# danisotelo/qm_door

Measured on AMD Instinct MI355X. Metric: MPC+WBC cycles/sec (AlienGo+Z1, N=100), higher is better.
Workload: dtype f64

## Files before the change

### qm_door_amd/csrc/kernels/aux_kernels.h

```cpp
#pragma once
#include "layout.h"
#include "lq_kernel.h"

namespace qmk {

__global__ void __launch_bounds__(64) input_weight_kernel(const ProblemR* P, const real* zeros, real* Rw) {
  __shared__ real J[12 * 12];
  __shared__ real RJ[12 * 12];
  const int lane = threadIdx.x;
  const ModelR& md = P->model;
  const int dd = lane < AD_DIRS ? lane : AD_DIRS - 1;
  const AdIn in{P->settings.initial_state, zeros, P->settings.initial_state, dd, 0.0_r};
  FlowOut<Du, Du3, Du3> f;
  BaseMotion2<Du, Du3> bm;
  centroidalSweep2<Du, Du3, Du3>(
      md, P->settings.gravity, in,
      [&](int c, Vec3<Du>, Vec3<Du3> v) {
        if (lane >= 3 && lane < 15) { const int j = lane - 3; J[(3 * c + 0) * 12 + j] = v.x.e; J[(3 * c + 1) * 12 + j] = v.y.e; J[(3 * c + 2) * 12 + j] = v.z.e; }
      },
      [&](Vec3<Du>, const Mat3<Du>&) { return Vec3<Du3>(); }, f, bm);
  __syncthreads();
  const real* Rt = P->settings.R_task;
  for (int e = lane; e < 144; e += 64) {
    const int i = e / 12, j = e % 12;
// ... 124 lines not shown
    for (int q = 0; q < NB; ++q) {
      const int iu0 = min(idx[q], Np - 1), iu1 = min(idx[q] + 1, Np - 1);
      const real* pl = isU ? Up + (size_t(inst) * Np + iu0) * 30 : Xp + (size_t(inst) * (Np + 1) + idx[q]) * 30;
      const real* pr = isU ? Up + (size_t(inst) * Np + iu1) * 30 : Xp + (size_t(inst) * (Np + 1) + min(idx[q] + 1, last)) * 30;
      l[q] = pl[c]; r[q] = pr[c];
    }
    const real x0v = (x0 && isX) ? x0[size_t(inst) * 30 + c] : 0.0_r;
#pragma unroll
    for (int q = 0; q < NB; ++q) { QM_KEEP(l[q]); QM_KEEP(r[q]); }
#pragma unroll
    for (int q = 0; q < NB; ++q) {
      const int k = k0 + q;
      const real v = alpha[q] * l[q] + (1.0_r - alpha[q]) * r[q];
      if (k <= Nn && isX) warmX[(size_t(inst) * (Nn + 1) + k) * 30 + c] = (k == 0 && x0) ? x0v : v;
      else if (k < Nn && isU) warmU[(size_t(inst) * Nn + k) * 30 + c] = v;
    }
  }
}

__global__ void __launch_bounds__(64) policy_eval_kernel(int batch, int N, const real* tgrid, const real* X, const real* U, const int* modes, const real* tEval,
                                                         real* xOut, real* uOut, int* modeOut) {
  const int inst = blockIdx.x, lane = threadIdx.x;
  if (inst >= batch) return;
  const real* tg = tgrid + size_t(inst) * (N + 1);
  const real t = tEval[inst];
  int idx; real alpha;
  timeSegmentWave(tg, N + 1, t, lane, idx, alpha);
  const int kMode = gridCountBelow(tg + 1, N, t, lane);
  if (lane < 30) {
    const real* xl = X + (size_t(inst) * (N + 1) + idx) * 30;
    xOut[size_t(inst) * 30 + lane] = alpha * xl[lane] + (1.0_r - alpha) * xl[30 + lane];
  } else if (lane >= 32 && lane < 62) {
    const int i = lane - 32, iu0 = min(idx, N - 1), iu1 = min(idx + 1, N - 1);
    const real* ul = U + (size_t(inst) * N + iu0) * 30; const real* ur = U + (size_t(inst) * N + iu1) * 30;
    uOut[size_t(inst) * 30 + i] = alpha * ul[i] + (1.0_r - alpha) * ur[i];
  } else if (lane == 63) {
    modeOut[inst] = modes[size_t(inst) * (N + 1) + kMode];
  }
}

}
```

### qm_door_amd/csrc/kernels/linesearch_kernel.h

```cpp
#pragma once
#include "layout.h"
#include "schedule_dev.h"
#include "sweep_dev.h"

namespace qmk {

struct LsArgs {
  const ProblemR* P;
  const real* Rw;
  int batch, N, K, lineSearch;
  const real* eeContact;
  const real* tgrid; const real* dtgrid; const int* nodePhase;
  const real* X; const real* U; const real* dX; const real* dU;
  const real* targetTimes; const real* targetStates;
  const int* schedNum; const real* schedTimes; const int* schedModes;
  const real* metrics;
  const real* instStats;
  const int* nodeMode;
  real* Xt; real* Ut;
  real* outT; real* outX; real* outU; int* outMode; real* outStats;
  int iteration;
  int trialInLds;
  int* done;
};

constexpr int LS_STATIC_LDS_BYTES = (3 * 256 + 8 + 1800) * int(sizeof(real)) + int(sizeof(ModelR)) + 256 * 4 + 256;
inline int lsTrialLdsBytes(int N, int threads = 256) {
  const int trials = (N + 1 <= threads / 2) ? 2 : 1;
  const long long need = (long long)trials * (2 * N + 1) * 30 * (long long)sizeof(real);
  return need + LS_STATIC_LDS_BYTES <= 160 * 1024 ? int(need) : 0;
}
inline int lsThreads(int B, int N, int cus) { return (B > cus && N + 1 <= 128) ? 128 : 256; }

struct DblIn {
  const real* x; const real* u; real dtS; const real* k1;
  __device__ __forceinline__ real hn(int i) const { return x[i] + dtS * k1[i]; }
  __device__ __forceinline__ real euler(int i) const { return x[9 + i] + dtS * k1[9 + i]; }
  __device__ __forceinline__ real q(int j) const { return x[12 + j] + dtS * u[12 + j]; }
  __device__ __forceinline__ real qd(int j) const { return u[12 + j]; }
  __device__ __forceinline__ Vec3<real> force(int c) const { return Vec3<real>(u[3 * c], u[3 * c + 1], u[3 * c + 2]); }
};

template <class WP> __device__ __attribute__((noinline)) void nodePerformance(const ModelR& md, const SettingsR& st, WP Qw, WP Rw, int weightStructure, const real* bc, const Schedule& sched, const real* tTimes, const real* tStates, const real* contact, int K, real t, real dt, int phase,
                                       bool terminal, const real* x, const real* u, const real* xnext, real& cost, real& dyn, real& eq, real* xnOut = nullptr) {
  QM_TICK_DECL;
  const int mode = sched.modes[phase];
  real eePosRef[3], eeQuatRef[4];
  eeReference(tTimes, tStates, K, t, eePosRef, eeQuatRef);
  real Ke = 0.0_r, fRef[3] = {0.0_r, 0.0_r, 0.0_r}, pEnv[3] = {0.0_r, 0.0_r, 0.0_r};
  if (contact && !terminal) { Ke = st.ee_contact_stiffness; eeContactReference(tTimes, contact, K, t, fRef, pEnv); }
// ... 112 lines not shown
#pragma unroll
    for (int q = 0; q < UN; ++q) { const int e = base + q * stride, ec = e < n ? e : first; xv[q] = x[ec]; dv[q] = dx[ec]; }
#pragma unroll
    for (int q = 0; q < UN; ++q) { QM_KEEP(xv[q]); QM_KEEP(dv[q]); }
#pragma unroll
    for (int q = 0; q < UN; ++q) { const int e = base + q * stride; if (e < n) out[e] = alpha == 0.0_r ? xv[q] : xv[q] + alpha * dv[q]; }
  }
}
__device__ __forceinline__ real sumSquaresStrided(const real* v, int n, int first, int stride) {
  constexpr int UN = 8;
  real s = 0.0_r;
  for (int base = first; base < n; base += UN * stride) {
    real t[UN];
#pragma unroll
    for (int q = 0; q < UN; ++q) { const int e = base + q * stride; t[q] = v[e < n ? e : first]; }
#pragma unroll
    for (int q = 0; q < UN; ++q) QM_KEEP(t[q]);
#pragma unroll
    for (int q = 0; q < UN; ++q) { const int e = base + q * stride; if (e < n) s += t[q] * t[q]; }
  }
  return s;
}

#ifdef QM_RICCATI_TIMING
#define QM_LS_CLOCK(slot) do { const unsigned long long n_ = clock64(); if (blockIdx.x == 0 && threadIdx.x == 0) qmk::qmRiccatiTicks[240 + (slot)] += n_ - lsClk; lsClk = n_; } while (0)
#else
#define QM_LS_CLOCK(slot)
#endif
#if defined(QM_LS_EXTERN) && !defined(QM_RICCATI_TIMING)
__global__ void __launch_bounds__(256) linesearch_kernel(LsArgs a);
#else
__global__ void __launch_bounds__(256) linesearch_kernel(LsArgs a) {
#ifdef QM_RICCATI_TIMING
  unsigned long long lsClk = clock64();
#endif
  __shared__ real red[3 * 256];
  __shared__ real ctl[8];
  __shared__ int structVotes[256];
  __shared__ ModelR mdS;
  __shared__ __attribute__((aligned(16))) real wQ[900], wR[900];
  const int inst = blockIdx.x, tid = threadIdx.x, nthr = blockDim.x;
  if (a.done[inst]) return;
  const int N = a.N;
  const SettingsR& st = a.P->settings;
  const real* tg = a.tgrid + size_t(inst) * (N + 1);
  const Schedule sched{a.schedNum[inst], a.schedTimes + size_t(inst) * QMGPU_MAX_EVENTS, a.schedModes + size_t(inst) * (QMGPU_MAX_EVENTS + 1)};
  const real* tTimes = a.targetTimes + size_t(inst) * a.K;
  const real* tStates = a.targetStates + size_t(inst) * a.K * QMGPU_NTARGET;
  const real* X = a.X + size_t(inst) * (N + 1) * 30; const real* U = a.U + size_t(inst) * N * 30;
  const real* dX = a.dX + size_t(inst) * (N + 1) * 30; const real* dU = a.dU + size_t(inst) * N * 30;
  const int half = (N + 1 <= nthr / 2) ? nthr / 2 : nthr;
  const int nTr = nthr / half, myTr = tid / half, ltid = tid - myTr * half;
  QM_DYNAMIC_LDS(trialLds);
  real* Xt = a.trialInLds ? trialLds + size_t(myTr) * (2 * N + 1) * 30 : a.Xt + (size_t(inst) * 2 + myTr) * (N + 1) * 30;
  real* Ut = a.trialInLds ? Xt + (N + 1) * 30 : a.Ut + (size_t(inst) * 2 + myTr) * N * 30;

  constexpr int MDW = (int(sizeof(ModelR) / 4) + 255) / 256;
  int mdw[2 * MDW];
  const int mdPer = nthr >= 256 ? MDW : 2 * MDW;
  real m0 = 0.0_r, d0 = 0.0_r, e0 = 0.0_r;
  {
    bool outside = false;
    real qv[4], rv4[4];
#pragma unroll
    for (int q4 = 0; q4 < 4; ++q4) { const int e = tid + q4 * nthr, ec = e < 900 ? e : tid; qv[q4] = st.Q[ec]; rv4[q4] = a.Rw[ec]; }
    {
      const int* src = reinterpret_cast<const int*>(&a.P->model);
#pragma unroll
      for (int w = 0; w < 2 * MDW; ++w) { const int e = tid + w * nthr; mdw[w] = (w < mdPer && e < int(sizeof(ModelR) / 4)) ? src[e] : 0; }
    }
    real mk[3] = {0.0_r, 0.0_r, 0.0_r};
    if (tid <= N) { const real* m = a.metrics + (size_t(inst) * (N + 1) + tid) * NODE_METRICS; mk[0] = m[0]; mk[1] = m[1]; mk[2] = m[2]; }
#pragma unroll
    for (int q4 = 0; q4 < 4; ++q4) { QM_KEEP(qv[q4]); QM_KEEP(rv4[q4]); }
#pragma unroll
    for (int w = 0; w < 2 * MDW; ++w) QM_KEEP(mdw[w]);
    QM_KEEP(mk[0]); QM_KEEP(mk[1]); QM_KEEP(mk[2]);
    if (tid <= N) { m0 = mk[0]; d0 = mk[1]; e0 = mk[2]; }
#pragma unroll
    for (int q4 = 0; q4 < 4; ++q4) {
      const int e = tid + q4 * nthr;
      if (e < 900) {
        const real q = qv[q4], r = rv4[q4];
        wQ[e] = q; wR[e] = r;
        const int i = e / 30, j = e - 30 * i;
        const bool legBlock = i >= 12 && i < 24 && j >= 12 && j < 24;
        outside = outside || (i != j && q != 0.0_r) || (i != j && !legBlock && r != 0.0_r);
      }
    }
    for (int e = tid + 4 * nthr; e < 900; e += nthr) {
      const real q = st.Q[e], r = a.Rw[e];
      wQ[e] = q; wR[e] = r;
      const int i = e / 30, j = e - 30 * i;
      const bool legBlock = i >= 12 && i < 24 && j >= 12 && j < 24;
      outside = outside || (i != j && q != 0.0_r) || (i != j && !legBlock && r != 0.0_r);
    }
    structVotes[tid] = outside ? 1 : 0;
  }
  {
    int* dst = reinterpret_cast<int*>(&mdS);
#pragma unroll
    for (int w = 0; w < 2 * MDW; ++w) { const int e = tid + w * nthr; if (w < mdPer && e < int(sizeof(ModelR) / 4)) dst[e] = mdw[w]; }
  }
  for (int k = tid + nthr; k <= N; k += nthr) { const real* m = a.metrics + (size_t(inst) * (N + 1) + k) * NODE_METRICS; m0 += m[0]; d0 += m[1]; e0 += m[2]; }
  red[tid] = m0; red[256 + tid] = d0; red[512 + tid] = e0;
  __syncthreads();
  if (tid == 0) {
    real s0 = 0, s1 = 0, s2 = 0;
    int dense = 0;
    const int nSum = N + 1 < nthr ? N + 1 : nthr;
    for (int i = 0; i < nSum; ++i) { s0 += red[i]; s1 += red[256 + i]; s2 += red[512 + i]; }
    for (int i = 0; i < nthr; ++i) dense |= structVotes[i];
    ctl[0] = s0; ctl[1] = sqrt(s1 + s2); ctl[7] = dense ? 0.0_r : 1.0_r;
  }
  __syncthreads();
  QM_LS_CLOCK(0);
  const real merit0 = ctl[0], viol0 = ctl[1];
  const int weightStructure = int(ctl[7]);
  const real armijo = a.instStats[size_t(inst) * 4 + 0];
  const real ricStatus = a.instStats[size_t(inst) * 4 + 1];

  real alpha = 1.0_r, merit1 = merit0, viol1 = viol0;
  int stepType = 0;
  bool accepted = false;
#pragma unroll 1
  for (int trial = 0; trial < (ricStatus == 0.0_r ? 64 : 0); ++trial) {
    const real alphaMine = myTr ? alpha * st.alpha_decay : alpha;
    axpyStrided(Xt, X, dX, alphaMine, (N + 1) * 30, ltid, half);
    axpyStrided(Ut, U, dU, alphaMine, N * 30, ltid, half);
    __syncthreads();
    QM_LS_CLOCK(1);
    real cs = 0.0_r, ds = 0.0_r, es = 0.0_r;
    for (int k = ltid; k <= N; k += half) {
      real c, d, e;
      const bool term = k == N;
      nodePerformance(mdS, st, QM_TO_LDS_PTR(real, wQ), QM_TO_LDS_PTR(real, wR), weightStructure, a.Rw + QM_RW_DERIVED, sched, tTimes, tStates, a.eeContact ? a.eeContact + size_t(inst) * a.K * 6 : nullptr, a.K, tg[k], a.dtgrid[size_t(inst) * (N + 1) + k], a.nodePhase[size_t(inst) * (N + 1) + k], term, Xt + k * 30, term ? Ut : Ut + k * 30, term ? Xt + k * 30 : Xt + (k + 1) * 30, c, d, e);
      cs += c; ds += d; es += e;
    }
    QM_LS_CLOCK(2);
    red[tid] = cs; red[256 + tid] = ds; red[512 + tid] = es;
    __syncthreads();
    QM_LS_CLOCK(3);
    if (tid == 0) {
      real acc = 0.0_r, accAlpha = alpha, m1 = merit0, v1 = viol0; int type = 0;
      for (int tr = 0; tr < nTr && acc == 0.0_r; ++tr) {
        const real al = tr ? alpha * st.alpha_decay : alpha;
        if (tr && al < st.alpha_min) break;
        real s0 = 0, s1 = 0, s2 = 0;
        const int nTrial = N + 1 < half ? N + 1 : half;
        for (int i = tr * half; i < tr * half + nTrial; ++i) { s0 += red[i]; s1 += red[256 + i]; s2 += red[512 + i]; }
        m1 = s0; v1 = sqrt(s1 + s2);
        bool ok;
        if (!a.lineSearch) { ok = true; type = 0; }
        else if (v1 > st.g_max) { ok = v1 < (1.0_r - st.gamma_c) * viol0; type = 1; }
        else if (v1 < st.g_min && viol0 < st.g_min && al * armijo < 0.0_r) { ok = m1 < merit0 + st.armijo_factor * al * armijo; type = 3; }
        else { ok = m1 < merit0 - st.gamma_c * viol0 || v1 < (1.0_r - st.gamma_c) * viol0; type = 2; }
        accAlpha = al;
        if (ok) acc = 1.0_r;
      }
      ctl[2] = m1; ctl[3] = v1; ctl[4] = acc; ctl[5] = real(type); ctl[6] = accAlpha;
    }
    __syncthreads();
    QM_LS_CLOCK(4);
    merit1 = ctl[2]; viol1 = ctl[3]; stepType = int(ctl[5]);
    accepted = ctl[4] != 0.0_r;
    const real lastAlpha = ctl[6];
    __syncthreads();
    if (accepted) { alpha = lastAlpha; break; }
    alpha = lastAlpha * st.alpha_decay;
    if (alpha < st.alpha_min) break;
  }
  if (!accepted) { alpha = 0.0_r; stepType = 4; merit1 = merit0; viol1 = viol0; }
  real* oX = a.outX + size_t(inst) * (N + 1) * 30; real* oU = a.outU + size_t(inst) * N * 30;
  axpyStrided(oX, X, dX, alpha, (N + 1) * 30, tid, nthr);
  axpyStrided(oU, U, dU, alpha, N * 30, tid, nthr);
  for (int k = tid; k <= N; k += nthr) { a.outT[size_t(inst) * (N + 1) + k] = tg[k]; a.outMode[size_t(inst) * (N + 1) + k] = a.nodeMode[size_t(inst) * (N + 1) + k]; }
  QM_LS_CLOCK(5);
  const real sx = sumSquaresStrided(dX, (N + 1) * 30, tid, nthr), su = sumSquaresStrided(dU, N * 30, tid, nthr);
  __syncthreads();
  red[tid] = sx; red[256 + tid] = su;
  __syncthreads();
  if (tid == 0) {
    real s0 = 0, s1 = 0;
    for (int i = 0; i < nthr; ++i) { s0 += red[i]; s1 += red[256 + i]; }
    int conv = 0;
    if (a.iteration + 1 >= st.sqp_iterations) conv = 1;
    else if (alpha < st.alpha_min) conv = 2;
    else if (fabs(merit1 - merit0) < st.cost_tol && viol1 < st.g_min) conv = 3;
    else if (alpha * sqrt(s0) < st.delta_tol && alpha * sqrt(s1) < st.delta_tol) conv = 4;
    if (ricStatus != 0.0_r && conv == 0) conv = 2;
    a.done[inst] = conv;
    if (a.outStats) {
      real* s = a.outStats + size_t(inst) * QMGPU_NSTATS;
      s[0] = merit0; s[1] = viol0; s[2] = merit1; s[3] = viol1; s[4] = alpha; s[5] = real(stepType); s[6] = armijo; s[7] = ricStatus;
      s[8] = real(a.iteration + 1); s[9] = real(conv);
    }
  }
  QM_LS_CLOCK(6);
}
#endif

}
```

### qm_door_amd/csrc/kernels/mpc_pipeline.h

```cpp
#pragma once
#include <vector>

#include "aux_kernels.h"
#include "ddp_kernel.h"
#include "gpu_rt.h"
#include "layout.h"
#include "linesearch_kernel.h"
#include "lq_kernel.h"
#include "riccati_kernel.h"

namespace qmk {

struct MpcBuffers {
  ProblemR* dP = nullptr;
  real *dRw = nullptr, *dZeros = nullptr;
  real *dTgrid = nullptr, *dDtgrid = nullptr, *dX = nullptr, *dU = nullptr, *dStages = nullptr, *dAdRows = nullptr, *dMetrics = nullptr, *dGains = nullptr, *ddX = nullptr, *ddU = nullptr;
  real *dXt = nullptr, *dUt = nullptr, *dInstStats = nullptr, *dDebug = nullptr;
  int *dStageNc = nullptr, *dNodeMode = nullptr, *dNodePhase = nullptr, *dDone = nullptr;
  real *dDdpX = nullptr, *dDdpU = nullptr, *dDdpMerit = nullptr;
  int cus = 256;
};

struct MpcIo {
  int batch, N, K, lineSearch;
  double dtD;
  const double *t0D, *timeGridD, *schedTimesD;
  const real *x0, *targetTimes, *targetStates;
  const int* schedNum; const real* schedTimes; const int* schedModes;
  const real *warmX, *warmU;
  real *outT, *outX, *outU; int* outMode; real* outStats;
  const real* eeContact;
  int algorithm;
};

template <class Alloc> inline void allocateMpcBuffers(MpcBuffers& m, size_t B, size_t N, Alloc&& alloc) {
  const size_t N1 = N + 1;
  auto R = [&](size_t n, bool scratch = true) { return static_cast<real*>(alloc(n, sizeof(real), scratch)); };
  auto I = [&](size_t n) { return static_cast<int*>(alloc(n, sizeof(int), true)); };
  m.dP = static_cast<ProblemR*>(alloc(1, sizeof(ProblemR), false));
  m.dRw = R(QM_RW_DOUBLES, false);
  m.dZeros = R(64, false);
  m.dTgrid = R(B * N1);
  m.dDtgrid = R(B * N1);
  m.dNodePhase = I(B * N1);
  m.dX = R(B * N1 * 30);
  m.dU = R(B * N * 30);
  m.dStages = R(B * N1 * STAGE_DOUBLES);
  m.dAdRows = R(B * N1 * AD_DOUBLES);
  m.dMetrics = R(B * N1 * NODE_METRICS);
  m.dGains = R(B * N * GAIN_DOUBLES);
  m.ddX = R(B * N1 * 30);
  m.ddU = R(B * N * 30);
  m.dXt = R(2 * B * N1 * 30);
  m.dUt = R(2 * B * N * 30);
  m.dInstStats = R(B * 4);
  m.dStageNc = I(B * N1);
  m.dNodeMode = I(B * N1);
  m.dDone = I(B);
  int dev = 0, cus = 0;
  if (hipGetDevice(&dev) == hipSuccess && hipDeviceGetAttribute(&cus, hipDeviceAttributeMultiprocessorCount, dev) == hipSuccess && cus > 0) m.cus = cus;
}

template <class Alloc> inline void ensureDdpBuffers(MpcBuffers& m, size_t B, size_t N, Alloc&& alloc) {
  if (m.dDdpX) return;
  m.dDdpX = static_cast<real*>(alloc(size_t(DDP_MAX_TRIALS) * B * (N + 1) * 30, sizeof(real), true));
  m.dDdpU = static_cast<real*>(alloc(size_t(DDP_MAX_TRIALS) * B * N * 30, sizeof(real), true));
  m.dDdpMerit = static_cast<real*>(alloc(size_t(DDP_MAX_TRIALS) * B * 2, sizeof(real), true));
}

inline hipError_t prepareMpcKernels() {
  const hipError_t e = QM_ALLOW_DYNAMIC_LDS(riccati_kernel<RICCATI_WAVES>, RICCATI_LDS_BYTES);
  return e != hipSuccess ? e : QM_ALLOW_DYNAMIC_LDS(linesearch_kernel, 160 * 1024 - LS_STATIC_LDS_BYTES);
}

inline void enqueueMpcKernels(hipStream_t s, const MpcBuffers& m, const MpcIo& io, int iterations, bool debugLq, hipEvent_t* ev) {
  const int B = io.batch, N = io.N;
  if (ev) (void)hipEventRecord(ev[0], s);
  for (int it = 0; it < iterations; ++it) {
    InitArgs ia{m.dP, B, N, io.dtD, io.t0D, io.timeGridD, io.schedTimesD, io.x0, it == 0 ? io.warmX : io.outX, it == 0 ? io.warmU : io.outU, io.schedNum, io.schedModes,
                m.dTgrid, m.dDtgrid, m.dNodePhase, m.dX, m.dU, it, m.dDone};
    QM_LAUNCH(mpc_init_kernel, B, 128, s, ia);
    LqArgs la{m.dP, m.dRw, B, N, io.K, m.dTgrid, m.dDtgrid, m.dNodePhase, m.dX, m.dU, io.targetTimes, io.targetStates, io.schedNum, io.schedTimes,
              io.schedModes, m.dZeros, m.dStages, m.dStageNc, m.dNodeMode, m.dMetrics, debugLq ? m.dDebug : nullptr, m.dAdRows, m.dDone, io.eeContact};
    QM_LAUNCH(ad_node_kernel, adGridFor(B * (N + 1)), 64, s, la);
    if (ev) (void)hipEventRecord(ev[6], s);
    QM_LAUNCH(lq_node_kernel, B * (N + 1), 64, s, la);
    if (ev) (void)hipEventRecord(ev[1], s);
    RiccatiArgs ra{B, N, m.dStages, m.dStageNc, m.dDtgrid, io.x0, m.dX, m.dGains, m.ddX, m.ddU, m.dInstStats, m.dDone};
    QM_LAUNCH_DYN(riccati_kernel<RICCATI_WAVES>, B, RICCATI_WAVES * 64, RICCATI_LDS_BYTES, s, ra);
    if (ev) (void)hipEventRecord(ev[2], s);
    LsArgs ls{m.dP, m.dRw, B, N, io.K, io.lineSearch, io.eeContact, m.dTgrid, m.dDtgrid, m.dNodePhase, m.dX, m.dU, m.ddX, m.ddU, io.targetTimes, io.targetStates, io.schedNum,
              io.schedTimes, io.schedModes, m.dMetrics, m.dInstStats, m.dNodeMode, m.dXt, m.dUt, io.outT, io.outX, io.outU, io.outMode, io.outStats, it, lsTrialLdsBytes(N, lsThreads(B, N, m.cus)) > 0, m.dDone};
    QM_LAUNCH_DYN(linesearch_kernel, B, lsThreads(B, N, m.cus), lsTrialLdsBytes(N, lsThreads(B, N, m.cus)), s, ls);
    if (ev) (void)hipEventRecord(ev[3], s);
  }
}

inline void enqueueDdpKernels(hipStream_t s, const MpcBuffers& m, const MpcIo& io, int trials, hipEvent_t* ev) {
  const int B = io.batch, N = io.N;
  if (ev) (void)hipEventRecord(ev[0], s);
  InitArgs ia{m.dP, B, N, io.dtD, io.t0D, io.timeGridD, io.schedTimesD, io.x0, io.warmX, io.warmU, io.schedNum, io.schedModes, m.dTgrid, m.dDtgrid, m.dNodePhase, m.dX, m.dU, 0, m.dDone};
  QM_LAUNCH(mpc_init_kernel, B, 128, s, ia);
  DdpArgs ra{m.dP, m.dRw, B, N, io.K, 0, io.eeContact, m.dTgrid, m.dDtgrid, m.dNodePhase, io.x0, m.dX, m.dU, io.targetTimes, io.targetStates, io.schedNum, io.schedTimes, io.schedModes,
             m.dStages, m.dStageNc, m.dGains, m.dX, m.dU, m.dDdpMerit};
  if (!io.warmX) QM_LAUNCH(ddp_rollout_kernel, (B + 63) / 64, 64, s, ra);
  LqArgs la{m.dP, m.dRw, B, N, io.K, m.dTgrid, m.dDtgrid, m.dNodePhase, m.dX, m.dU, io.targetTimes, io.targetStates, io.schedNum, io.schedTimes,
            io.schedModes, m.dZeros, m.dStages, m.dStageNc, m.dNodeMode, m.dMetrics, nullptr, m.dAdRows, m.dDone, io.eeContact};
  QM_LAUNCH(ad_node_kernel, adGridFor(B * (N + 1)), 64, s, la);
  if (ev) (void)hipEventRecord(ev[6], s);
  QM_LAUNCH(lq_node_kernel, B * (N + 1), 64, s, la);
  if (ev) (void)hipEventRecord(ev[1], s);
  RiccatiArgs ri{B, N, m.dStages, m.dStageNc, m.dDtgrid, io.x0, m.dX, m.dGains, m.ddX, m.ddU, m.dInstStats, m.dDone};
  QM_LAUNCH_DYN(riccati_kernel<RICCATI_WAVES>, B, RICCATI_WAVES * 64, RICCATI_LDS_BYTES, s, ri);
  if (ev) (void)hipEventRecord(ev[2], s);
  ra.trials = trials; ra.Xout = m.dDdpX; ra.Uout = m.dDdpU;
// ... 14 lines not shown
```

### qm_door_amd/csrc/kernels/schedule_dev.h

```cpp
#pragma once
#include "problem_r.h"
#include "gpu_rt.h"

namespace qmk {

struct Schedule {
  int numEvents;
  const real* eventTimes;
  const int* modes;
};

__device__ __forceinline__ int nodePhaseAt(const Schedule& s, real t) {
  int i = 0;
  while (i < s.numEvents && s.eventTimes[i] <= t) ++i;
  return i;
}
__device__ __forceinline__ bool contactOf(int mode, int leg) { return (mode >> (3 - leg)) & 1; }

__device__ __forceinline__ void cubic(real t0, real p0, real v0, real t1, real p1, real v1, real t, real& pos, real& vel) {
  const real dt = t1 - t0, dp = p1 - p0, dv = v1 - v0;
  const real c1 = v0 * dt, c2 = -(3.0_r * v0 + dv) * dt + 3.0_r * dp, c3 = (2.0_r * v0 + dv) * dt - 2.0_r * dp;
  const real tn = (t - t0) / dt;
  pos = ((c3 * tn + c2) * tn + c1) * tn + p0;
  vel = ((3.0_r * c3 * tn + 2.0_r * c2) * tn + c1) / dt;
// ... 31 lines not shown
  int lb = 0;
  for (int base = 0; base < K; base += 64) {
    const int i = base + lane;
    const bool below = i < K && times[i < K ? i : 0] < t;
    const unsigned long long m = qmBallot(below);
    lb += qmPopCount(m);
    if (m != ~0ull) break;
  }
  return lb;
}
__device__ __forceinline__ void timeSegmentWave(const real* times, int K, real t, int lane, int& index, real& alpha) {
  if (K <= 1) { index = 0; alpha = 1.0_r; return; }
  const int lb = gridCountBelow(times, K, t, lane);
  const int interval = lb - 1, last = K - 1;
  if (interval < 0) { index = 0; alpha = 1.0_r; }
  else if (interval >= last) { index = max(last - 1, 0); alpha = 0.0_r; }
  else {
    const real len = times[interval + 1] - times[interval];
    index = interval;
    alpha = (len > 2.0_r * REAL_EPS) ? (times[interval + 1] - t) / len : 1.0_r;
  }
}

__device__ inline void eeReference(const real* times, const real* states, int K, real t, real pos[3], real quat[4]) {
  int idx; real alpha;
  timeSegment(times, K, t, idx, alpha);
  const real* lhs = states + size_t(idx) * QMGPU_NTARGET;
  if (K <= 1) {
    for (int i = 0; i < 3; ++i) pos[i] = lhs[30 + i];
    for (int i = 0; i < 4; ++i) quat[i] = lhs[33 + i];
    return;
  }
  const real* rhs = lhs + QMGPU_NTARGET;
  for (int i = 0; i < 3; ++i) pos[i] = alpha * lhs[30 + i] + (1.0_r - alpha) * rhs[30 + i];
  const real tt = 1.0_r - alpha;
  const real* a = lhs + 33; const real* b = rhs + 33;
  const real d = a[0] * b[0] + a[1] * b[1] + a[2] * b[2] + a[3] * b[3];
  const real absD = fabs(d);
  real s0, s1;
  if (absD >= 1.0_r - REAL_EPS) { s0 = 1.0_r - tt; s1 = tt; }
  else { const real theta = acos(absD), sinTheta = sin(theta); s0 = sin((1.0_r - tt) * theta) / sinTheta; s1 = sin(tt * theta) / sinTheta; }
  if (d < 0) s1 = -s1;
  for (int i = 0; i < 4; ++i) quat[i] = s0 * a[i] + s1 * b[i];
}
__device__ inline void eeContactReference(const real* times, const real* contact, int K, real t, real fref[3], real env[3]) {
  int idx; real alpha;
// ... 29 lines not shown
```

### qm_door_amd/csrc/qmgpu_api.hip

```cpp
#include <algorithm>
#include <cstdio>
#include <cstring>
#include <string>
#include <vector>

#include "../../include/qmgpu.h"
#include "host/host_error.h"
#include "kernels/mpc_pipeline.h"
#include "kernels/wbc_kernel.h"
#include "kernels/frontend_kernel.h"
#include "mpc32.h"

using namespace qmhost;
using namespace qmk;

#define HIP_CHECK(expr)                                                                                       \
  do {                                                                                                        \
    hipError_t e_ = (expr);                                                                                   \
    if (e_ != hipSuccess) throw HipFailure(std::string(#expr) + " failed: " + hipGetErrorString(e_));         \
  } while (0)

struct DeviceGuard {
  int prev = -1;
  explicit DeviceGuard(int device) {
    if (hipGetDevice(&prev) != hipSuccess) prev = -1;
    if (prev != device) HIP_CHECK(hipSetDevice(device));
    else prev = -1;
  }
  ~DeviceGuard() { if (prev >= 0) (void)hipSetDevice(prev); }
  DeviceGuard(const DeviceGuard&) = delete;
  DeviceGuard& operator=(const DeviceGuard&) = delete;
};

struct qmgpu_context {
  int device = 0, maxBatch = 0, maxNodes = 0;
  hipStream_t ownStream = nullptr, stream = nullptr;
  hipStream_t wbcStream = nullptr;
  hipEvent_t evPolicy = nullptr, evWbc = nullptr;
  bool overlap = false, wbcPending = false;
  qmgpu_problem hostProblem;
  int dtype = QMGPU_F64;
  MpcBuffers m;
  qmk32::Mpc32* m32 = nullptr;
  double *dPolX = nullptr, *dPolU = nullptr;
  int* dPolMode = nullptr;
  qmgpu_gait* dGaits = nullptr;
  std::vector<void*> allocations;
  bool timing = false, debugLq = false;
  static constexpr int kRing = 256;
  hipEvent_t ring[kRing][7];
  int ringKind[kRing];
  long callCount = 0;
  hipEvent_t* ev = nullptr;
  double lastMs[5] = {0, 0, 0, 0, 0};
  int lastBatch = 0, lastN = 0;

  std::vector<std::pair<void*, size_t>> scratch;
  template <class T> T* alloc(size_t count, bool isScratch = true) {
    void* p = nullptr;
    HIP_CHECK(hipMalloc(&p, count * sizeof(T)));
    allocations.push_back(p);
    if (isScratch) scratch.emplace_back(p, count * sizeof(T));
    return static_cast<T*>(p);
  }
};

static void checkTopology(const qmgpu_model& m) {
  bool ok = m.parent[0] == -1;
// ... 14 lines not shown
  return qmgpu_create_ex(problem, device, max_batch, max_nodes, QMGPU_F64, out);
}

int qmgpu_create_ex(const qmgpu_problem* problem, int device, int max_batch, int max_nodes, int dtype, qmgpu_handle* out) {
  if (!problem || !out || max_batch < 1 || max_nodes < 1 || (dtype != QMGPU_F64 && dtype != QMGPU_F32)) return setError(QMGPU_ERR_INVALID_ARGUMENT, "bad arguments to qmgpu_create");
  *out = nullptr;
  qmgpu_context* ctx = nullptr;
  const int st = guarded([&]() {
    checkTopology(problem->model);
    int count = 0;
    if (hipGetDeviceCount(&count) != hipSuccess || count <= 0) throw NoDevice("no HIP device visible; qm_door_amd has no CPU execution path");
    if (device < 0 || device >= count) throw NoDevice("HIP device index out of range");
    DeviceGuard onDevice(device);
    ctx = new qmgpu_context();
    for (auto& set : ctx->ring) for (auto& e : set) e = nullptr;
    ctx->device = device; ctx->maxBatch = max_batch; ctx->maxNodes = max_nodes; ctx->hostProblem = *problem; ctx->dtype = dtype;
    HIP_CHECK(hipStreamCreate(&ctx->ownStream));
    ctx->stream = ctx->ownStream;
    const size_t B = size_t(max_batch), N1 = size_t(max_nodes) + 1, N = size_t(max_nodes);
    qmgpu_context* const owner = ctx;
    auto rawAlloc = [owner](size_t count, size_t elem, bool scratch) { return static_cast<void*>(owner->alloc<char>(count * elem, scratch)); };
    if (dtype == QMGPU_F64) allocateMpcBuffers(ctx->m, B, N, rawAlloc);
    else { ctx->m.dP = ctx->alloc<qmgpu_problem>(1, false); ctx->m.dRw = ctx->alloc<double>(qmk::QM_RW_DOUBLES, false); ctx->m.dZeros = ctx->alloc<double>(64, false); }
    ctx->dPolX = ctx->alloc<double>(B * 30);
    ctx->dPolU = ctx->alloc<double>(B * 30);
    ctx->dPolMode = ctx->alloc<int>(B);
    HIP_CHECK(hipMemcpy(ctx->m.dP, problem, sizeof(qmgpu_problem), hipMemcpyHostToDevice));
    HIP_CHECK(hipMemsetAsync(ctx->m.dZeros, 0, 64 * sizeof(double), ctx->stream));
    for (auto& set : ctx->ring) for (auto& e : set) HIP_CHECK(hipEventCreate(&e));
    ctx->ev = ctx->ring[0];
    HIP_CHECK(QM_ALLOW_DYNAMIC_LDS(wbc_kernel, WBC_LDS_BYTES));
    HIP_CHECK(prepareMpcKernels());
    QM_LAUNCH(input_weight_kernel, 1, 64, ctx->stream, ctx->m.dP, ctx->m.dZeros, ctx->m.dRw);
    HIP_CHECK(hipGetLastError());
    if (dtype == QMGPU_F32) {
      ctx->m32 = qmk32::create(*problem, max_batch, max_nodes, ctx->stream, rawAlloc);
      if (!ctx->m32) throw HipFailure("fp32 MPC path could not be created");
    }
    HIP_CHECK(hipStreamSynchronize(ctx->stream));
  });
  if (st != QMGPU_OK) {
    if (ctx) {
      int prev = -1;
      const bool sw = hipGetDevice(&prev) == hipSuccess && prev != ctx->device && hipSetDevice(ctx->device) == hipSuccess;
      for (void* p : ctx->allocations) hipFree(p);
      for (auto& set : ctx->ring) for (auto& e : set) if (e) hipEventDestroy(e);
      if (ctx->ownStream) hipStreamDestroy(ctx->ownStream);
      if (sw) hipSetDevice(prev);
      qmk32::destroy(ctx->m32);
// ... 133 lines not shown
    HIP_CHECK(hipGetLastError());
  });
}

int qmgpu_enable_debug(qmgpu_handle h, int enable) {
  if (!h) return setError(QMGPU_ERR_INVALID_ARGUMENT, "null handle");
  return guarded([&]() { if (!h) throw std::invalid_argument("null handle"); DeviceGuard onDevice(h->device);
    if (enable && h->dtype != QMGPU_F64) throw std::invalid_argument("the per-node LQ dump exists in the fp64 path only");
    if (enable && !h->m.dDebug) h->m.dDebug = h->alloc<double>(size_t(h->maxBatch) * (h->maxNodes + 1) * DBG_DOUBLES);
    h->debugLq = enable != 0;
  });
}

static void checkMpcArgs(qmgpu_handle h, const qmgpu_mpc_args* a) {
  if (!h || !a) throw std::invalid_argument("null argument");
  if (a->batch < 1 || a->num_nodes < 1 || a->num_target_knots < 1) throw std::invalid_argument("batch, num_nodes and num_target_knots must be positive");
  if (a->batch > h->maxBatch || a->num_nodes > h->maxNodes) throw CapacityError("batch / num_nodes exceed the capacity given to qmgpu_create");
  if (h->dtype == QMGPU_F32 && a->num_target_knots > QMGPU_F32_MAX_TARGET_KNOTS) throw CapacityError("an fp32 handle stages at most QMGPU_F32_MAX_TARGET_KNOTS target knots per instance");
  if (!a->x0 || !a->target_times || !a->target_states || !a->sched_num_events || !a->sched_event_times || !a->sched_modes) throw std::invalid_argument("missing MPC input pointer");
  if (!a->time_grid && !a->t0) throw std::invalid_argument("either t0 or time_grid is required");
  if (!a->out_t || !a->out_x || !a->out_u || !a->out_mode) throw std::invalid_argument("missing MPC output pointer");
}

static void enqueueMpc(qmgpu_handle h, const qmgpu_mpc_args* a) {
  const int iterations = h->hostProblem.settings.sqp_iterations > 1 ? h->hostProblem.settings.sqp_iterations : 1;
  hipEvent_t* ev = h->timing ? h->ev : nullptr;
  if (a->algorithm != QMGPU_ALG_SQP && a->algorithm != QMGPU_ALG_DDP) throw std::invalid_argument("unknown qmgpu_mpc_args::algorithm");
  const int trials = ddpTrialCount(h->hostProblem.settings.ddp_min_step, h->hostProblem.settings.ddp_max_step);
  if (h->dtype == QMGPU_F32) {
    if (!qmk32::enqueue(h->m32, h->stream, a, h->hostProblem.settings.dt, iterations, trials, ev)) throw HipFailure("fp32 MPC launch failed");
  } else if (a->algorithm == QMGPU_ALG_DDP) {
    ensureDdpBuffers(h->m, size_t(h->maxBatch), size_t(h->maxNodes), [&](size_t count, size_t elem, bool scratch) { return static_cast<void*>(h->alloc<char>(count * elem, scratch)); });
    const MpcIo io{a->batch, a->num_nodes, a->num_target_knots, a->line_search, h->hostProblem.settings.dt, a->t0, a->time_grid, a->sched_event_times, a->x0, a->target_times,
                   a->target_states, a->sched_num_events, a->sched_event_times, a->sched_modes, a->warm_x, a->warm_u, a->out_t, a->out_x, a->out_u, a->out_mode, a->out_stats, a->ee_contact_ref,
                   a->algorithm};
    enqueueDdpKernels(h->stream, h->m, io, trials, ev);
  } else {
    const MpcIo io{a->batch, a->num_nodes, a->num_target_knots, a->line_search, h->hostProblem.settings.dt, a->t0, a->time_grid, a->sched_event_times, a->x0, a->target_times,
                   a->target_states, a->sched_num_events, a->sched_event_times, a->sched_modes, a->warm_x, a->warm_u, a->out_t, a->out_x, a->out_u, a->out_mode, a->out_stats, a->ee_contact_ref, a->algorithm};
    enqueueMpcKernels(h->stream, h->m, io, iterations, h->debugLq, ev);
  }
  HIP_CHECK(hipGetLastError());
  h->lastBatch = a->batch; h->lastN = a->num_nodes;
}

static void enqueueWbc(qmgpu_handle h, const qmgpu_wbc_args* w, hipStream_t stream) {
  if (!w || w->batch < 1) throw std::invalid_argument("bad WBC arguments");
  if (w->batch > h->maxBatch) throw CapacityError("WBC batch exceeds the capacity given to qmgpu_create");
  if (!w->state_desired || !w->input_desired || !w->rbd_measured || !w->mode || !w->period || !w->time || !w->input_last || !w->out) throw std::invalid_argument("missing WBC pointer");
  static_assert(sizeof(unsigned long long) == sizeof(uint64_t), "working-set words");
  WbcArgs wa{h->m.dP, w->batch, w->variant, w->state_desired, w->input_desired, w->rbd_measured, w->mode, w->period, w->time, w->input_last, w->out, w->out_status, w->ee_force,
             reinterpret_cast<unsigned long long*>(w->working_set)};
  QM_LAUNCH_DYN(wbc_kernel, w->batch, WBC_THREADS, WBC_LDS_BYTES, stream, wa);
  HIP_CHECK(hipGetLastError());
}

static void beginTiming(qmgpu_handle h) {
  if (h->timing) h->ev = h->ring[h->callCount % qmgpu_context::kRing];
}
static void finishTiming(qmgpu_handle h, bool mpc, bool wbc) {
  if (!h->timing) return;
  h->ringKind[h->callCount % qmgpu_context::kRing] = (mpc ? 1 : 0) | (wbc ? 2 : 0);
  ++h->callCount;
// ... 63 lines not shown
    enqueueWbc(h, args, h->stream);
    if (h->timing) HIP_CHECK(hipEventRecord(h->ev[5], h->stream));
    finishTiming(h, false, true);
  });
}

int qmgpu_warm_start_batch(qmgpu_handle h, int batch, int prev_nodes, const double* prev_grid, const double* prev_X, const double* prev_U, int new_nodes,
                           const double* new_grid, const double* x0, double* warm_x, double* warm_u) {
  if (!h || !prev_grid || !prev_X || !prev_U || !new_grid || !warm_x || !warm_u || batch < 1 || prev_nodes < 1 || new_nodes < 1)
    return setError(QMGPU_ERR_INVALID_ARGUMENT, "bad warm-start arguments");
  if (warm_x == prev_X || warm_u == prev_U) return setError(QMGPU_ERR_INVALID_ARGUMENT, "warm-start outputs must not alias the previous solution");
  return guarded([&]() { if (!h) throw std::invalid_argument("null handle"); DeviceGuard onDevice(h->device);
    QM_LAUNCH(warm_start_kernel, batch, 256, h->stream, batch, prev_nodes, prev_grid, prev_X, prev_U, new_nodes, new_grid, x0, warm_x, warm_u);
    HIP_CHECK(hipGetLastError());
  });
}

int qmgpu_cycle_batch(qmgpu_handle h, const qmgpu_mpc_args* mpc, const double* t_eval, qmgpu_wbc_args* wbc) {
  if (!h || !t_eval || !wbc) return setError(QMGPU_ERR_INVALID_ARGUMENT, "null argument");
  return guarded([&]() { if (!h) throw std::invalid_argument("null handle"); DeviceGuard onDevice(h->device);
    checkMpcArgs(h, mpc);
    if (wbc->batch != mpc->batch) throw std::invalid_argument("MPC and WBC batch sizes differ");
    beginTiming(h);
    enqueueMpc(h, mpc);
    joinWbc(h);
    QM_LAUNCH(policy_eval_kernel, mpc->batch, 64, h->stream, mpc->batch, mpc->num_nodes, mpc->out_t, mpc->out_x, mpc->out_u, mpc->out_mode, t_eval, h->dPolX, h->dPolU,
              h->dPolMode);
    qmgpu_wbc_args w = *wbc;
    w.state_desired = h->dPolX; w.input_desired = h->dPolU; w.mode = h->dPolMode;
    hipStream_t ws = h->stream;
    if (h->overlap) {
      HIP_CHECK(hipEventRecord(h->evPolicy, h->stream));
      HIP_CHECK(hipStreamWaitEvent(h->wbcStream, h->evPolicy, 0));
      ws = h->wbcStream;
    }
    if (h->timing) HIP_CHECK(hipEventRecord(h->ev[4], ws));
    enqueueWbc(h, &w, ws);
    if (h->timing) HIP_CHECK(hipEventRecord(h->ev[5], ws));
    if (h->overlap) { HIP_CHECK(hipEventRecord(h->evWbc, ws)); h->wbcPending = true; }
    finishTiming(h, true, true);
  });
}

int qmgpu_debug_get_lq(qmgpu_handle h, int instance, int node, double* A, double* B, double* b, double* Q, double* R, double* q, double* r, double* C, double* D, double* e,
                       int32_t* nc) {
  if (!h) return setError(QMGPU_ERR_INVALID_ARGUMENT, "null handle");
  return guarded([&]() { if (!h) throw std::invalid_argument("null handle"); DeviceGuard onDevice(h->device);
    if (!h->debugLq || !h->m.dDebug) throw std::invalid_argument("call qmgpu_enable_debug(h, 1) before the solve");
    if (instance < 0 || instance >= h->lastBatch || node < 0 || node > h->lastN) throw std::invalid_argument("instance / node out of range");
    HIP_CHECK(hipStreamSynchronize(h->stream));
    std::vector<double> rec(DBG_DOUBLES);
    const size_t idx = size_t(instance) * (h->lastN + 1) + node;
    HIP_CHECK(hipMemcpy(rec.data(), h->m.dDebug + idx * DBG_DOUBLES, DBG_DOUBLES * sizeof(double), hipMemcpyDeviceToHost));
    int ncv = 0;
    HIP_CHECK(hipMemcpy(&ncv, h->m.dStageNc + idx, sizeof(int), hipMemcpyDeviceToHost));
    auto cp = [&](double* dst, int off, int n) { if (dst) std::memcpy(dst, rec.data() + off, n * sizeof(double)); };
    cp(A, DBG_A, 900); cp(B, DBG_B, 900); cp(b, DBG_b, 30); cp(Q, DBG_Q, 900); cp(R, DBG_R, 900); cp(q, DBG_q, 30); cp(r, DBG_r, 30);
    cp(C, DBG_C, 16 * 30); cp(D, DBG_D, 16 * 30); cp(e, DBG_e, 16);
// ... 42 lines not shown
```

Before: 158,400.

## Fuse policy evaluation into line-search kernel and double-buffer policy outputs

The policy interpolation at t_eval now runs inside the last SQP iteration's line-search kernel, in its final wave, so the separate policy_eval_kernel launch is dropped for f64 SQP. Policy output buffers are double-buffered, which lets the WBC join move after the MPC enqueue and lets the next MPC overlap the previous WBC. The line search also prefetches the sum-of-squares loads early and copies the accepted trajectory from LDS instead of recomputing the axpy. Risks include extra register pressure and added complexity in the done-instance early-exit path.

```diff
diff --git a/qm_door_amd/csrc/kernels/aux_kernels.h b/qm_door_amd/csrc/kernels/aux_kernels.h
--- a/qm_door_amd/csrc/kernels/aux_kernels.h
+++ b/qm_door_amd/csrc/kernels/aux_kernels.h
@@ -170,21 +170,8 @@
                                                          real* xOut, real* uOut, int* modeOut) {
   const int inst = blockIdx.x, lane = threadIdx.x;
   if (inst >= batch) return;
-  const real* tg = tgrid + size_t(inst) * (N + 1);
-  const real t = tEval[inst];
-  int idx; real alpha;
-  timeSegmentWave(tg, N + 1, t, lane, idx, alpha);
-  const int kMode = gridCountBelow(tg + 1, N, t, lane);
-  if (lane < 30) {
-    const real* xl = X + (size_t(inst) * (N + 1) + idx) * 30;
-    xOut[size_t(inst) * 30 + lane] = alpha * xl[lane] + (1.0_r - alpha) * xl[30 + lane];
-  } else if (lane >= 32 && lane < 62) {
-    const int i = lane - 32, iu0 = min(idx, N - 1), iu1 = min(idx + 1, N - 1);
-    const real* ul = U + (size_t(inst) * N + iu0) * 30; const real* ur = U + (size_t(inst) * N + iu1) * 30;
-    uOut[size_t(inst) * 30 + i] = alpha * ul[i] + (1.0_r - alpha) * ur[i];
-  } else if (lane == 63) {
-    modeOut[inst] = modes[size_t(inst) * (N + 1) + kMode];
-  }
+  policyEvalWave(tgrid + size_t(inst) * (N + 1), X + size_t(inst) * (N + 1) * 30, U + size_t(inst) * N * 30, modes + size_t(inst) * (N + 1), N, tEval[inst], lane,
+                 xOut + size_t(inst) * 30, uOut + size_t(inst) * 30, modeOut + inst);
 }
 
 }
diff --git a/qm_door_amd/csrc/kernels/linesearch_kernel.h b/qm_door_amd/csrc/kernels/linesearch_kernel.h
--- a/qm_door_amd/csrc/kernels/linesearch_kernel.h
+++ b/qm_door_amd/csrc/kernels/linesearch_kernel.h
@@ -22,10 +22,14 @@
   int iteration;
   int trialInLds;
   int* done;
+  const real* tEval; real* polX; real* polU; int* polMode;
 };
 
 constexpr int LS_STATIC_LDS_BYTES = (3 * 256 + 8 + 1800) * int(sizeof(real)) + int(sizeof(ModelR)) + 256 * 4 + 256;
 inline int lsTrialLdsBytes(int N, int threads = 256) {
+#ifdef QM_LS_TRIAL_IN_HBM
+  return 0;
+#endif
   const int trials = (N + 1 <= threads / 2) ? 2 : 1;
   const long long need = (long long)trials * (2 * N + 1) * 30 * (long long)sizeof(real);
   return need + LS_STATIC_LDS_BYTES <= 160 * 1024 ? int(need) : 0;
@@ -184,6 +188,23 @@
   return s;
 }
 
+__device__ __forceinline__ void squaresRequest(const real* v, int n, int first, int base, int stride, real (&t)[8]) {
+#pragma unroll
+  for (int q = 0; q < 8; ++q) { const int e = base + q * stride; t[q] = v[e < n ? e : first]; }
+}
+__device__ __forceinline__ void squaresAdd(int n, int base, int stride, real (&t)[8], real& s) {
+#pragma unroll
+  for (int q = 0; q < 8; ++q) QM_KEEP(t[q]);
+#pragma unroll
+  for (int q = 0; q < 8; ++q) { const int e = base + q * stride; if (e < n) s += t[q] * t[q]; }
+}
+
+#ifdef QMGPU_HOST_EMULATION
+#define QM_WG_GLOBAL_BARRIER() __syncthreads()
+#else
+#define QM_WG_GLOBAL_BARRIER() do { __builtin_amdgcn_fence(__ATOMIC_RELEASE, "workgroup"); __syncthreads(); __builtin_amdgcn_fence(__ATOMIC_ACQUIRE, "workgroup"); } while (0)
+#endif
+
 #ifdef QM_RICCATI_TIMING
 #define QM_LS_CLOCK(slot) do { const unsigned long long n_ = clock64(); if (blockIdx.x == 0 && threadIdx.x == 0) qmk::qmRiccatiTicks[240 + (slot)] += n_ - lsClk; lsClk = n_; } while (0)
 #else
@@ -202,8 +223,14 @@
   __shared__ ModelR mdS;
   __shared__ __attribute__((aligned(16))) real wQ[900], wR[900];
   const int inst = blockIdx.x, tid = threadIdx.x, nthr = blockDim.x;
-  if (a.done[inst]) return;
   const int N = a.N;
+  const int polWave = (nthr >> 6) - 1, lane = tid & 63;
+  if (a.done[inst]) {
+    if (a.tEval && (tid >> 6) == polWave)
+      policyEvalWave(a.outT + size_t(inst) * (N + 1), a.outX + size_t(inst) * (N + 1) * 30, a.outU + size_t(inst) * N * 30, a.outMode + size_t(inst) * (N + 1), N, a.tEval[inst], lane,
+                     a.polX + size_t(inst) * 30, a.polU + size_t(inst) * 30, a.polMode + inst);
+    return;
+  }
   const SettingsR& st = a.P->settings;
   const real* tg = a.tgrid + size_t(inst) * (N + 1);
   const Schedule sched{a.schedNum[inst], a.schedTimes + size_t(inst) * QMGPU_MAX_EVENTS, a.schedModes + size_t(inst) * (QMGPU_MAX_EVENTS + 1)};
@@ -221,6 +248,8 @@
   int mdw[2 * MDW];
   const int mdPer = nthr >= 256 ? MDW : 2 * MDW;
   real m0 = 0.0_r, d0 = 0.0_r, e0 = 0.0_r;
+  const int nX = (N + 1) * 30, nU = N * 30;
+  real sx = 0.0_r, su = 0.0_r;
   {
     bool outside = false;
     real qv[4], rv4[4];
@@ -233,12 +262,19 @@
     }
     real mk[3] = {0.0_r, 0.0_r, 0.0_r};
     if (tid <= N) { const real* m = a.metrics + (size_t(inst) * (N + 1) + tid) * NODE_METRICS; mk[0] = m[0]; mk[1] = m[1]; mk[2] = m[2]; }
+    real tx[8], tu[8];
+    squaresRequest(dX, nX, tid, tid, nthr, tx); squaresRequest(dU, nU, tid, tid, nthr, tu);
 #pragma unroll
     for (int q4 = 0; q4 < 4; ++q4) { QM_KEEP(qv[q4]); QM_KEEP(rv4[q4]); }
 #pragma unroll
     for (int w = 0; w < 2 * MDW; ++w) QM_KEEP(mdw[w]);
     QM_KEEP(mk[0]); QM_KEEP(mk[1]); QM_KEEP(mk[2]);
     if (tid <= N) { m0 = mk[0]; d0 = mk[1]; e0 = mk[2]; }
+    squaresAdd(nX, tid, nthr, tx, sx); squaresAdd(nU, tid, nthr, tu, su);
+    for (int base = tid + 8 * nthr; base < nX; base += 8 * nthr) {
+      squaresRequest(dX, nX, tid, base, nthr, tx); squaresRequest(dU, nU, tid, base, nthr, tu);
+      squaresAdd(nX, base, nthr, tx, sx); squaresAdd(nU, base, nthr, tu, su);
+    }
 #pragma unroll
     for (int q4 = 0; q4 < 4; ++q4) {
       const int e = tid + q4 * nthr;
@@ -283,7 +319,7 @@
   const real ricStatus = a.instStats[size_t(inst) * 4 + 1];
 
   real alpha = 1.0_r, merit1 = merit0, viol1 = viol0;
-  int stepType = 0;
+  int stepType = 0, accTrial = 0;
   bool accepted = false;
 #pragma unroll 1
   for (int trial = 0; trial < (ricStatus == 0.0_r ? 64 : 0); ++trial) {
@@ -304,7 +340,7 @@
     __syncthreads();
     QM_LS_CLOCK(3);
     if (tid == 0) {
-      real acc = 0.0_r, accAlpha = alpha, m1 = merit0, v1 = viol0; int type = 0;
+      real acc = 0.0_r, accAlpha = alpha, m1 = merit0, v1 = viol0; int type = 0, accTr = 0;
       for (int tr = 0; tr < nTr && acc == 0.0_r; ++tr) {
         const real al = tr ? alpha * st.alpha_decay : alpha;
         if (tr && al < st.alpha_min) break;
@@ -317,14 +353,14 @@
         else if (v1 > st.g_max) { ok = v1 < (1.0_r - st.gamma_c) * viol0; type = 1; }
         else if (v1 < st.g_min && viol0 < st.g_min && al * armijo < 0.0_r) { ok = m1 < merit0 + st.armijo_factor * al * armijo; type = 3; }
         else { ok = m1 < merit0 - st.gamma_c * viol0 || v1 < (1.0_r - st.gamma_c) * viol0; type = 2; }
-        accAlpha = al;
+        accAlpha = al; accTr = tr;
         if (ok) acc = 1.0_r;
       }
-      ctl[2] = m1; ctl[3] = v1; ctl[4] = acc; ctl[5] = real(type); ctl[6] = accAlpha;
+      ctl[2] = m1; ctl[3] = v1; ctl[4] = acc; ctl[5] = real(type + 8 * accTr); ctl[6] = accAlpha;
     }
     __syncthreads();
     QM_LS_CLOCK(4);
-    merit1 = ctl[2]; viol1 = ctl[3]; stepType = int(ctl[5]);
+    merit1 = ctl[2]; viol1 = ctl[3]; stepType = int(ctl[5]) & 7; accTrial = int(ctl[5]) >> 3;
     accepted = ctl[4] != 0.0_r;
     const real lastAlpha = ctl[6];
     __syncthreads();
@@ -333,15 +369,21 @@
     if (alpha < st.alpha_min) break;
   }
   if (!accepted) { alpha = 0.0_r; stepType = 4; merit1 = merit0; viol1 = viol0; }
-  real* oX = a.outX + size_t(inst) * (N + 1) * 30; real* oU = a.outU + size_t(inst) * N * 30;
-  axpyStrided(oX, X, dX, alpha, (N + 1) * 30, tid, nthr);
-  axpyStrided(oU, U, dU, alpha, N * 30, tid, nthr);
+  real* oX = a.outX + size_t(inst) * nX; real* oU = a.outU + size_t(inst) * nU;
+  if (accepted && a.trialInLds) {
+    const real* accX = trialLds + size_t(accTrial) * (2 * N + 1) * 30; const real* accU = accX + nX;
+    for (int e = tid; e < nX; e += nthr) oX[e] = accX[e];
+    for (int e = tid; e < nU; e += nthr) oU[e] = accU[e];
+  } else {
+    axpyStrided(oX, X, dX, alpha, nX, tid, nthr);
+    axpyStrided(oU, U, dU, alpha, nU, tid, nthr);
+  }
   for (int k = tid; k <= N; k += nthr) { a.outT[size_t(inst) * (N + 1) + k] = tg[k]; a.outMode[size_t(inst) * (N + 1) + k] = a.nodeMode[size_t(inst) * (N + 1) + k]; }
   QM_LS_CLOCK(5);
-  const real sx = sumSquaresStrided(dX, (N + 1) * 30, tid, nthr), su = sumSquaresStrided(dU, N * 30, tid, nthr);
-  __syncthreads();
   red[tid] = sx; red[256 + tid] = su;
-  __syncthreads();
+  QM_WG_GLOBAL_BARRIER();
+  if (a.tEval && (tid >> 6) == polWave)
+    policyEvalWave(a.outT + size_t(inst) * (N + 1), oX, oU, a.outMode + size_t(inst) * (N + 1), N, a.tEval[inst], lane, a.polX + size_t(inst) * 30, a.polU + size_t(inst) * 30, a.polMode + inst);
   if (tid == 0) {
     real s0 = 0, s1 = 0;
     for (int i = 0; i < nthr; ++i) { s0 += red[i]; s1 += red[256 + i]; }
diff --git a/qm_door_amd/csrc/kernels/mpc_pipeline.h b/qm_door_amd/csrc/kernels/mpc_pipeline.h
--- a/qm_door_amd/csrc/kernels/mpc_pipeline.h
+++ b/qm_door_amd/csrc/kernels/mpc_pipeline.h
@@ -32,6 +32,8 @@
   const real* eeContact;
   int algorithm;
 };
+
+struct PolicyOut { const real* tEval; real* x; real* u; int* mode; };
 
 template <class Alloc> inline void allocateMpcBuffers(MpcBuffers& m, size_t B, size_t N, Alloc&& alloc) {
   const size_t N1 = N + 1;
@@ -73,7 +75,7 @@
   return e != hipSuccess ? e : QM_ALLOW_DYNAMIC_LDS(linesearch_kernel, 160 * 1024 - LS_STATIC_LDS_BYTES);
 }
 
-inline void enqueueMpcKernels(hipStream_t s, const MpcBuffers& m, const MpcIo& io, int iterations, bool debugLq, hipEvent_t* ev) {
+inline void enqueueMpcKernels(hipStream_t s, const MpcBuffers& m, const MpcIo& io, int iterations, bool debugLq, hipEvent_t* ev, const PolicyOut* pol = nullptr) {
   const int B = io.batch, N = io.N;
   if (ev) (void)hipEventRecord(ev[0], s);
   for (int it = 0; it < iterations; ++it) {
@@ -90,7 +92,9 @@
     QM_LAUNCH_DYN(riccati_kernel<RICCATI_WAVES>, B, RICCATI_WAVES * 64, RICCATI_LDS_BYTES, s, ra);
     if (ev) (void)hipEventRecord(ev[2], s);
     LsArgs ls{m.dP, m.dRw, B, N, io.K, io.lineSearch, io.eeContact, m.dTgrid, m.dDtgrid, m.dNodePhase, m.dX, m.dU, m.ddX, m.ddU, io.targetTimes, io.targetStates, io.schedNum,
-              io.schedTimes, io.schedModes, m.dMetrics, m.dInstStats, m.dNodeMode, m.dXt, m.dUt, io.outT, io.outX, io.outU, io.outMode, io.outStats, it, lsTrialLdsBytes(N, lsThreads(B, N, m.cus)) > 0, m.dDone};
+              io.schedTimes, io.schedModes, m.dMetrics, m.dInstStats, m.dNodeMode, m.dXt, m.dUt, io.outT, io.outX, io.outU, io.outMode, io.outStats, it, lsTrialLdsBytes(N, lsThreads(B, N, m.cus)) > 0, m.dDone,
+              nullptr, nullptr, nullptr, nullptr};
+    if (pol && it == iterations - 1) { ls.tEval = pol->tEval; ls.polX = pol->x; ls.polU = pol->u; ls.polMode = pol->mode; }
     QM_LAUNCH_DYN(linesearch_kernel, B, lsThreads(B, N, m.cus), lsTrialLdsBytes(N, lsThreads(B, N, m.cus)), s, ls);
     if (ev) (void)hipEventRecord(ev[3], s);
   }
diff --git a/qm_door_amd/csrc/kernels/schedule_dev.h b/qm_door_amd/csrc/kernels/schedule_dev.h
--- a/qm_door_amd/csrc/kernels/schedule_dev.h
+++ b/qm_door_amd/csrc/kernels/schedule_dev.h
@@ -77,6 +77,22 @@
   }
 }
 
+__device__ __forceinline__ void policyEvalWave(const real* tg, const real* X, const real* U, const int* modes, int N, real t, int lane, real* xOut, real* uOut, int* modeOut) {
+  int idx; real alpha;
+  timeSegmentWave(tg, N + 1, t, lane, idx, alpha);
+  const int kMode = gridCountBelow(tg + 1, N, t, lane);
+  if (lane < 30) {
+    const real* xl = X + size_t(idx) * 30;
+    xOut[lane] = alpha * xl[lane] + (1.0_r - alpha) * xl[30 + lane];
+  } else if (lane >= 32 && lane < 62) {
+    const int i = lane - 32, iu0 = min(idx, N - 1), iu1 = min(idx + 1, N - 1);
+    const real* ul = U + size_t(iu0) * 30; const real* ur = U + size_t(iu1) * 30;
+    uOut[i] = alpha * ul[i] + (1.0_r - alpha) * ur[i];
+  } else if (lane == 63) {
+    modeOut[0] = modes[kMode];
+  }
+}
+
 __device__ inline void eeReference(const real* times, const real* states, int K, real t, real pos[3], real quat[4]) {
   int idx; real alpha;
   timeSegment(times, K, t, idx, alpha);
diff --git a/qm_door_amd/csrc/qmgpu_api.hip b/qm_door_amd/csrc/qmgpu_api.hip
--- a/qm_door_amd/csrc/qmgpu_api.hip
+++ b/qm_door_amd/csrc/qmgpu_api.hip
@@ -42,8 +42,9 @@
   int dtype = QMGPU_F64;
   MpcBuffers m;
   qmk32::Mpc32* m32 = nullptr;
-  double *dPolX = nullptr, *dPolU = nullptr;
-  int* dPolMode = nullptr;
+  double *dPolX[2] = {nullptr, nullptr}, *dPolU[2] = {nullptr, nullptr};
+  int* dPolMode[2] = {nullptr, nullptr};
+  int polSet = 0;
   qmgpu_gait* dGaits = nullptr;
   std::vector<void*> allocations;
   bool timing = false, debugLq = false;
@@ -104,9 +105,7 @@
     auto rawAlloc = [owner](size_t count, size_t elem, bool scratch) { return static_cast<void*>(owner->alloc<char>(count * elem, scratch)); };
     if (dtype == QMGPU_F64) allocateMpcBuffers(ctx->m, B, N, rawAlloc);
     else { ctx->m.dP = ctx->alloc<qmgpu_problem>(1, false); ctx->m.dRw = ctx->alloc<double>(qmk::QM_RW_DOUBLES, false); ctx->m.dZeros = ctx->alloc<double>(64, false); }
-    ctx->dPolX = ctx->alloc<double>(B * 30);
-    ctx->dPolU = ctx->alloc<double>(B * 30);
-    ctx->dPolMode = ctx->alloc<int>(B);
+    for (int set = 0; set < 2; ++set) { ctx->dPolX[set] = ctx->alloc<double>(B * 30); ctx->dPolU[set] = ctx->alloc<double>(B * 30); ctx->dPolMode[set] = ctx->alloc<int>(B); }
     HIP_CHECK(hipMemcpy(ctx->m.dP, problem, sizeof(qmgpu_problem), hipMemcpyHostToDevice));
     HIP_CHECK(hipMemsetAsync(ctx->m.dZeros, 0, 64 * sizeof(double), ctx->stream));
     for (auto& set : ctx->ring) for (auto& e : set) HIP_CHECK(hipEventCreate(&e));
@@ -286,7 +285,7 @@
   if (!a->out_t || !a->out_x || !a->out_u || !a->out_mode) throw std::invalid_argument("missing MPC output pointer");
 }
 
-static void enqueueMpc(qmgpu_handle h, const qmgpu_mpc_args* a) {
+static void enqueueMpc(qmgpu_handle h, const qmgpu_mpc_args* a, const PolicyOut* pol = nullptr) {
   const int iterations = h->hostProblem.settings.sqp_iterations > 1 ? h->hostProblem.settings.sqp_iterations : 1;
   hipEvent_t* ev = h->timing ? h->ev : nullptr;
   if (a->algorithm != QMGPU_ALG_SQP && a->algorithm != QMGPU_ALG_DDP) throw std::invalid_argument("unknown qmgpu_mpc_args::algorithm");
@@ -302,7 +301,7 @@
   } else {
     const MpcIo io{a->batch, a->num_nodes, a->num_target_knots, a->line_search, h->hostProblem.settings.dt, a->t0, a->time_grid, a->sched_event_times, a->x0, a->target_times,
                    a->target_states, a->sched_num_events, a->sched_event_times, a->sched_modes, a->warm_x, a->warm_u, a->out_t, a->out_x, a->out_u, a->out_mode, a->out_stats, a->ee_contact_ref, a->algorithm};
-    enqueueMpcKernels(h->stream, h->m, io, iterations, h->debugLq, ev);
+    enqueueMpcKernels(h->stream, h->m, io, iterations, h->debugLq, ev, pol);
   }
   HIP_CHECK(hipGetLastError());
   h->lastBatch = a->batch; h->lastN = a->num_nodes;
@@ -412,18 +411,22 @@
     checkMpcArgs(h, mpc);
     if (wbc->batch != mpc->batch) throw std::invalid_argument("MPC and WBC batch sizes differ");
     beginTiming(h);
-    enqueueMpc(h, mpc);
-    joinWbc(h);
-    QM_LAUNCH(policy_eval_kernel, mpc->batch, 64, h->stream, mpc->batch, mpc->num_nodes, mpc->out_t, mpc->out_x, mpc->out_u, mpc->out_mode, t_eval, h->dPolX, h->dPolU,
-              h->dPolMode);
+    const int set = h->polSet;
+    h->polSet ^= 1;
+    const bool policyInLineSearch = h->dtype == QMGPU_F64 && mpc->algorithm == QMGPU_ALG_SQP;
+    const PolicyOut pol{t_eval, h->dPolX[set], h->dPolU[set], h->dPolMode[set]};
+    enqueueMpc(h, mpc, policyInLineSearch ? &pol : nullptr);
+    if (!policyInLineSearch)
+      QM_LAUNCH(policy_eval_kernel, mpc->batch, 64, h->stream, mpc->batch, mpc->num_nodes, mpc->out_t, mpc->out_x, mpc->out_u, mpc->out_mode, t_eval, pol.x, pol.u, pol.mode);
     qmgpu_wbc_args w = *wbc;
-    w.state_desired = h->dPolX; w.input_desired = h->dPolU; w.mode = h->dPolMode;
+    w.state_desired = pol.x; w.input_desired = pol.u; w.mode = pol.mode;
     hipStream_t ws = h->stream;
     if (h->overlap) {
       HIP_CHECK(hipEventRecord(h->evPolicy, h->stream));
       HIP_CHECK(hipStreamWaitEvent(h->wbcStream, h->evPolicy, 0));
       ws = h->wbcStream;
     }
+    joinWbc(h);
     if (h->timing) HIP_CHECK(hipEventRecord(h->ev[4], ws));
     enqueueWbc(h, &w, ws);
     if (h->timing) HIP_CHECK(hipEventRecord(h->ev[5], ws));
```

Result: no change. 158,300 (-0.0%).
